# pjmikkol/bwtc

Measured on NVIDIA B200. Metric: forward BWT MB/s (SA+BWT, 32 MiB blocks), higher is better.
Workload: dtype u8 text / u32 ranks / u64 sort keys (integer)

## Files before the change

### bwtc_b200/__init__.py

```python
from __future__ import annotations

import ctypes
import os
from typing import List, Optional, Sequence

import numpy as np

_HERE = os.path.dirname(os.path.abspath(__file__))
LIB_PATH = os.path.join(_HERE, "libbwtc_cuda.so")
GEN_LIB_PATH = os.path.join(_HERE, "libbwtc_gen.so")
INTEGRATION_LIB_PATH = os.path.join(_HERE, "libbwtc_integration.so")

MAX_ROUNDS = 40
MAX_BLOCK = 0x7FFFFFFD
SCRATCH_BYTES_PER_SUFFIX = 40
SCRATCH_FIXED_BYTES = 8 << 20
ECORRUPT = -6
EVERIFY = -7
FLAG_VERIFIED = 1 << 6
FLAG_CORRUPT = 1 << 7
FLAG_SA = 1 << 8


class BwtcCudaUnavailable(RuntimeError):
    """The CUDA engine library is not built / not loadable.  There is no fallback path."""


class BwtcCudaError(RuntimeError):
    def __init__(self, code: int, msg: str, blocks: Optional[List[int]] = None):
        super().__init__(f"bwtc_cuda error {code}: {msg}")
        self.code = code
        self.blocks = blocks


class Stats(ctypes.Structure):

    _fields_ = [
        ("n_suffixes", ctypes.c_uint32),
        ("sigma", ctypes.c_uint32),
        ("bits_per_char", ctypes.c_uint32),
        ("chars_round0", ctypes.c_uint32),
        ("key_bytes_round0", ctypes.c_uint32),
        ("rounds", ctypes.c_uint32),
        ("live", ctypes.c_uint32 * MAX_ROUNDS),
        ("passes", ctypes.c_uint32 * MAX_ROUNDS),
        ("prefix_len", ctypes.c_uint32 * MAX_ROUNDS),
        ("kernel_launches", ctypes.c_uint64),
        ("algorithmic_bytes", ctypes.c_uint64),
        ("gpu_ms", ctypes.c_float),
        ("sort_ms", ctypes.c_float),
        ("sort_bytes", ctypes.c_uint64),
        ("sort_launches", ctypes.c_uint32),
        ("sort0_launches", ctypes.c_uint32),
        ("sort0_bytes", ctypes.c_uint64),
        ("sort0_ms", ctypes.c_float),
        ("flags", ctypes.c_uint32),
        ("batch_blocks", ctypes.c_uint32),
    ]

    def as_dict(self) -> dict:
        r = int(self.rounds)
        return {
            "n_suffixes": int(self.n_suffixes), "sigma": int(self.sigma), "bits_per_char": int(self.bits_per_char),
            "chars_round0": int(self.chars_round0), "key_bytes_round0": int(self.key_bytes_round0), "rounds": r,
            "live": [int(self.live[i]) for i in range(r)], "passes": [int(self.passes[i]) for i in range(r)],
            "prefix_len": [int(self.prefix_len[i]) for i in range(r)],
            "kernel_launches": int(self.kernel_launches), "algorithmic_bytes": int(self.algorithmic_bytes),
            "gpu_ms": float(self.gpu_ms), "sort_ms": float(self.sort_ms), "sort_bytes": int(self.sort_bytes),
            "sort_launches": int(self.sort_launches), "sort0_launches": int(self.sort0_launches),
            "sort0_bytes": int(self.sort0_bytes), "sort0_ms": float(self.sort0_ms), "flags": int(self.flags),
            "batch_blocks": int(self.batch_blocks),
        }


# ... 517 lines not shown
```

### bwtc_b200/csrc/bwt_engine.cu

```cuda
#include "../../include/bwtc_cuda.h"
#include "bwt_kernels.cuh"
#include "ibwt_kernels.cuh"

#include <algorithm>
#include <atomic>
#include <chrono>
#include <cmath>
#include <condition_variable>
#include <cstdarg>
#include <cstdio>
#include <cstdlib>
#include <cstring>
#include <deque>
#include <memory>
#include <mutex>
#include <thread>
#include <unordered_map>
#include <vector>

using namespace bwtc_b200;

namespace {

constexpr int RS_BLOCK = BWTC_RS_BLOCK;
// ... 48 lines not shown
  int wait_mode = 0;
  uint32_t cap = 0;
  size_t max_rs_tiles = 0, max_aux_tiles = 0;
  uint8_t* d_in = nullptr;
  uint8_t* d_text = nullptr;
  uint8_t* d_out = nullptr;
  uint32_t* d_rank = nullptr;
  void* d_keys[2] = {nullptr, nullptr};
  uint32_t* d_idx[2] = {nullptr, nullptr};
  uint8_t* d_aux[2] = {nullptr, nullptr};
  uint32_t* d_scat = nullptr;
  uint32_t* d_zero = nullptr;
  uint32_t* d_status = nullptr;
  uint32_t* d_tilecnt = nullptr;
  uint32_t* d_LF = nullptr;
  uint32_t* d_livebits = nullptr;
  uint32_t* d_ktab = nullptr;
  LookupParams* d_lookup = nullptr;
  LookupParams* h_lookup = nullptr;
  LadderState* d_state = nullptr;
  LadderState* h_state = nullptr;
  unsigned long long* d_wtab = nullptr;
  uint32_t* d_bhist = nullptr;
  const uint8_t** d_bptr = nullptr;
  int32_t* d_sa = nullptr;
  uint32_t* h_small = nullptr;
  uint8_t* h_batch = nullptr;
  cudaEvent_t ev_begin = nullptr, ev_end = nullptr;
  std::vector<cudaEvent_t> ev_pool;
  int timing_detail = 0;
  int static_tiles = 1;
  int lb_watchdog = 0;
  int debug_fake_watchdog = 0;
  int debug_reverse_tiles = 0;
  int verify = 0;
  int debug_corrupt_out = 0;
  uint32_t debug_corrupt_lf = 0;
  int64_t debug_corrupt_sa = -1;
  int d2h_kernel = 0;
  int d2h_ctas = 16;
  int debug_skip_copies = 0;
  int ladder_first = 2, ladder_more = 4;
  int use_radix9 = 0;
  uint32_t status_row_words = 256;
  int use_partial = 1;
  int use_gram = 1;
  int twopass = 0;
  int hybrid2 = 0;
  uint32_t rerank_pf_tiles = 0;
  int use_lazy = 1;
  uint32_t lazy_min_suffixes = 4u << 20;
  double lazy_max_live = 0.09;
  double lazy_max_repeats = 32.0;
  int use_seg = 1;
  int use_batch = 1;
  int use_pack_pred = 1;
  uint32_t aux_min_suffixes = 96u << 20;
  int bucket_min_windows = 3;
  uint64_t rerank_window_bytes = 72ull << 20;
  uint32_t force_chars = 0, force_keybytes = 0;
  uint32_t debug_max_rounds = 0;
  int last_cur = 0;
  RerankParams rr0;
  bwtc_cuda_stats stats;
  char err[512];
  uint32_t* d_ctrl() const { return d_zero; }
  uint32_t* d_hist() const { return d_zero + CTR_WORDS; }
  unsigned long long* d_tstate() const { return reinterpret_cast<unsigned long long*>(d_zero + CTR_WORDS + HIST_WORDS); }
  uint32_t* h_ctrl() const { return h_small; }
  uint32_t* h_hist() const { return h_small + CTR_WORDS; }
  uint32_t* h_LF() const { return h_small + CTR_WORDS + HIST_WORDS; }
};

#define CK(ctx, call)                                                                              \
  do {                                                                                             \
    cudaError_t e_ = (call);                                                                       \
    if (e_ != cudaSuccess) {                                                                       \
      set_err((ctx)->err, "CUDA error %s at %s:%d: %s", cudaGetErrorName(e_), __FILE__, __LINE__,  \
              cudaGetErrorString(e_));                                                             \
      return BWTC_CUDA_ECUDA;                                                                      \
    }                                                                                              \
  } while (0)

namespace {

template <typename KeyT, int IPT, bool IOTA, bool AUX, int RB = 8>
int set_pass_attr(bwtc_cuda_ctx* ctx) {
  CK(ctx, cudaFuncSetAttribute(k_radix_pass<KeyT, RS_BLOCK, IPT, IOTA, AUX, RB>, cudaFuncAttributeMaxDynamicSharedMemorySize,
                               (int)RadixPassSmem<KeyT, RS_BLOCK, IPT, AUX, RB>::bytes));
  return 0;
}

void ctx_free(bwtc_cuda_ctx* c) {
  if (!c) return;
  cudaSetDevice(c->device);
  if (c->stream) cudaStreamSynchronize(c->stream);
  cudaFree(c->d_in); cudaFree(c->d_text); cudaFree(c->d_out); cudaFree(c->d_rank);
  cudaFree(c->d_keys[0]); cudaFree(c->d_keys[1]); cudaFree(c->d_idx[0]); cudaFree(c->d_idx[1]);
  cudaFree(c->d_zero); cudaFree(c->d_status); cudaFree(c->d_LF); cudaFree(c->d_wtab); cudaFree(c->d_tilecnt); cudaFree(c->d_scat);
  cudaFree(c->d_bhist); cudaFree(c->d_bptr); cudaFree(c->d_aux[0]); cudaFree(c->d_aux[1]);
  cudaFree(c->d_state); cudaFree(c->d_livebits); cudaFree(c->d_ktab); cudaFree(c->d_lookup); cudaFree(c->d_sa);
  if (c->h_lookup) cudaFreeHost(c->h_lookup);
  if (c->h_batch) cudaFreeHost(c->h_batch);
  if (c->h_small) cudaFreeHost(c->h_small);
  if (c->h_state) cudaFreeHost(c->h_state);
  if (c->h_ring) cudaFreeHost(c->h_ring);
// ... 57 lines not shown
      chars = cmax64;
      for (uint32_t c = 1; c <= cmax64; ++c) {
        const double p0 = std::ceil(((double)c * b + blk_bits) / 8.0) * ((uint64_t)c * b + blk_bits > 32 ? 1.1 : 1.0);
        const double L = 1.0 - std::exp(-(double)N * std::exp2(-H0 * (double)c));
        const double cost = p0 + L * (npd + 2.0);
        if (cost < best - 1e-9) { best = cost; chars = c; }
      }
      const uint32_t np = div_up((uint64_t)chars * b + blk_bits, 8);
      const uint32_t cfull = (8 * np - blk_bits) / b;
      const uint32_t cap = ((uint64_t)chars * b + blk_bits <= 32) ? cmax32 : cmax64;
      chars = cfull < cap ? cfull : cap;
      keybytes = ((uint64_t)chars * b + blk_bits <= 32) ? 4 : 8;
    }
  }
  pl->has_memory = true;
  pl->live_pred = 1.0;
  pl->repeats = HUGE_VAL;
  if (!(ctx->force_chars || ctx->force_keybytes)) {
    double q2 = 0.0;
    for (int c = 0; c < 256; ++c)
      if (present[c] && count[c]) { const double q = (double)count[c] / total; q2 += q * q; }
    const double samples = pair_stats[1];
    const double all_pairs = samples * (samples - 1.0) * 0.5;
    const double expected = all_pairs * std::pow(q2, 8.0);
    pl->has_memory = (H0 < 1e-3) || samples < 64.0 || (pair_stats[0] > 8.0 * expected + 16.0);
    if (!pl->has_memory) pl->live_pred = 1.0 - std::exp(-(double)N * std::exp2(-H0 * (double)chars));
    if (samples >= 64.0) pl->repeats = pair_stats[0] / all_pairs * (double)N;
  }
  pl->sigma = sigma;
  pl->bits = b;
  pl->chars = chars;
  pl->keybytes = keybytes;
  pl->npass = div_up((uint64_t)chars * b + blk_bits, 8);
  pl->rb = 8;
  if (ctx->use_radix9 && keybytes == 8 && div_up((uint64_t)chars * b + blk_bits, 9) < pl->npass) {
    pl->rb = 9;
    pl->npass = div_up((uint64_t)chars * b + blk_bits, 9);
  }
  {
    const uint32_t covered = std::min<uint32_t>(pl->rb * pl->npass, keybytes * 8u);
    const uint32_t used = chars * b + blk_bits;
    uint32_t r = (ctx->use_partial && blk_bits == 0 && covered > used) ? covered - used : 0u;
    if (r >= b) r = b - 1u;
    if (chars >= 64u) r = 0;
    pl->rbits = r;
  }
  pl->pp.rbits = pl->rbits;
  pl->pp.bits = b;
  pl->pp.chars = chars;
  pl->pp.nblocks = 1;
  pl->pp.stride = 0;
}

uint32_t rerank_windows(const bwtc_cuda_ctx* ctx, uint32_t N, uint32_t m) {
  if ((uint64_t)m * 4 < (uint64_t)N) return 1;
  uint64_t w = ((uint64_t)N * 4 + ctx->rerank_window_bytes - 1) / ctx->rerank_window_bytes;
  if (w < 1) w = 1;
  if (!ctx->bucket_min_windows && w > 8) w = 8;
  if (w > MAX_RERANK_WINDOWS) w = MAX_RERANK_WINDOWS;
  return (uint32_t)w;
}

uint32_t rerank_launches(const bwtc_cuda_ctx* ctx, uint32_t N, uint32_t m) {
  const uint32_t w = rerank_windows(ctx, N, m);
  return (ctx->bucket_min_windows && w >= (uint32_t)ctx->bucket_min_windows) ? 1u : w;
}

inline bool dbg_any(const bwtc_cuda_ctx* ctx) { return ctx->debug_max_rounds != 0; }

inline uint32_t tile_slot(const bwtc_cuda_ctx* ctx, uint32_t ticket_word) {
  if (!ctx->static_tiles) return ticket_word;
  return ctx->debug_reverse_tiles ? CTR_STATIC_REV : CTR_STATIC;
}

inline uint32_t* status_rows(const bwtc_cuda_ctx* ctx, int p) {
  return ctx->d_status + ((size_t)p * (ctx->max_rs_tiles + LB_PAD_ROWS) + LB_PAD_ROWS) * ctx->status_row_words;
}

struct PassTimer {
  bwtc_cuda_ctx* ctx;
  size_t used = 0;
  int begin() {
    if (!ctx->timing_detail) return 0;
    if (used + 2 > ctx->ev_pool.size()) return 0;
    CK(ctx, cudaEventRecord(ctx->ev_pool[used], ctx->stream));
    return 0;
  }
  int end() {
    if (!ctx->timing_detail) return 0;
    if (used + 2 > ctx->ev_pool.size()) return 0;
    CK(ctx, cudaEventRecord(ctx->ev_pool[used + 1], ctx->stream));
    used += 2;
    return 0;
  }
};

template <typename KeyT, int IPT, bool AUX, int RB = 8>
int run_sort_impl(bwtc_cuda_ctx* ctx, uint32_t m, uint32_t pass_mask, bool first_iota, uint32_t iota_top, int* cur_io,
                  PassTimer* pt, uint32_t* passes_done, uint32_t pack_bits, uint32_t topshift, uint32_t pred_mask) {
  constexpr uint32_t TILE = RS_BLOCK * IPT;
  const uint32_t tiles = div_up(m, TILE);
  const size_t smem = RadixPassSmem<KeyT, RS_BLOCK, IPT, AUX, RB>::bytes;
  int cur = *cur_io;
  bool iota = first_iota;
  uint32_t done = 0;
  for (int p = 0; p < MAX_PASSES; ++p) {
// ... 391 lines not shown
  } else {
    const uint8_t last = J.h_in ? J.h_in[N - 1] : *h_last;
    J.last = last;
    J.present[last] = true;
    count[last] += 1;
  }
  double pair_stats[2];
  memcpy(pair_stats, ctx->h_LF() + 256, 16);
  plan_round0(ctx, count, J.present, N, pair_stats, &J.pl, J.blk_bits);
  if (bs) { J.pl.pp.nblocks = bs->nblocks; J.pl.pp.stride = J.bstride; }
  J.ep.nblocks = bs ? bs->nblocks : 1u;
  J.ep.stride = J.bstride;
  J.ep.text = J.d_text;
  J.ep.out = J.d_dst;
  J.ep.lastch = ctx->d_LF + LF_PARK;
  J.ep.N = N;
  J.ep.block_mode = J.block_mode ? 1 : 0;
  J.ep.sa = J.sa;
  S.sigma = J.pl.sigma;
  S.bits_per_char = J.pl.bits;
  S.chars_round0 = J.pl.chars;
  S.key_bytes_round0 = J.pl.keybytes;
  J.a_launches = S.kernel_launches;
  J.a_bytes = S.algorithmic_bytes;
  return 0;
}

int verify_forward(bwtc_cuda_ctx* ctx, const Job& J);
int verify_sa(bwtc_cuda_ctx* ctx, const Job& J);

int64_t phase_sort(bwtc_cuda_ctx* ctx, Job& J) {
  ctx->lb_watchdog = 0;
  if (cudaSetDevice(ctx->device) != cudaSuccess) {
    set_err(ctx->err, "cudaSetDevice(%d) failed", ctx->device);
    return BWTC_CUDA_ECUDA;
  }
  cudaStream_t st = ctx->stream;
  bwtc_cuda_stats& S = ctx->stats;
  const BatchSpec* bs = J.bs;
  const uint32_t N = J.N, n = J.n;
  const Round0Plan& pl = J.pl;
  const EmitParams& ep = J.ep;
  const uint8_t* d_text = J.d_text;
  PassTimer pt{ctx};
  S.kernel_launches = J.a_launches;
  S.algorithmic_bytes = J.a_bytes;
  S.sort_bytes = S.sort0_bytes = 0;
  S.sort_launches = S.sort0_launches = 0;
  CK(ctx, cudaMemsetAsync(ctx->d_zero, 0, (size_t)CTR_STICKY * 4, st));
  CK(ctx, cudaMemsetAsync(ctx->d_state, 0, sizeof(LadderState), st));
  CK(ctx, cudaMemsetAsync(ctx->d_LF + LF_PARK, 0, (size_t)(LF_WORDS - LF_PARK) * 4, st));

  const uint32_t rs_tile0 = pl.keybytes == 4 ? RS_TILE32 : RS_TILE64;
  const uint32_t all0 = (1u << pl.npass) - 1u;
  if (zero_round_state(ctx, N, N, rs_tile0, all0, pl.rb)) return BWTC_CUDA_ECUDA;
  {
    const uint32_t ptiles = div_up(N, AUX_TILE);
    const int grid = (int)(ptiles < (uint32_t)(ctx->sm_count * 4) ? ptiles : (uint32_t)(ctx->sm_count * 4));
    uint32_t hist_mask = 0;
    DeriveParams dp;
    dp.count = 0;
    const uint32_t keybits = pl.chars * pl.bits;
    const uint32_t rbits = pl.rbits;
    uint32_t regular_mask = 0;
    for (uint32_t p = 0; p < pl.npass; ++p) {
      int rep = -1;
      const uint32_t rb = pl.rb;
      const bool full_p = (rb * p >= rbits) && (rb * p - rbits + rb <= keybits);
      if (full_p) regular_mask |= 1u << p;
      if (full_p && N > 64 && !bs)
        for (uint32_t r = 0; r < p; ++r)
          if (((hist_mask >> r) & (regular_mask >> r) & 1u) && (rb * (p - r)) % pl.bits == 0) { rep = (int)r; break; }
      if (rep < 0) {
        hist_mask |= 1u << p;
      } else {
        dp.p[dp.count] = (uint8_t)p;
        dp.r[dp.count] = (uint8_t)rep;
        dp.t[dp.count] = (uint8_t)(pl.rb * (p - (uint32_t)rep) / pl.bits);
        dp.count++;
      }
    }
    GramParams gp;
    gp.npass = 0;
    bool use_gram = ctx->use_gram && !bs && N > 64 && (pl.bits == 6 || pl.bits == 3) && keybits >= (uint32_t)GRAM_BITS;
    if (use_gram) {
      const uint32_t W = (uint32_t)GRAM_BITS / pl.bits;
      for (uint32_t p = 0; p < pl.npass && use_gram; ++p) {
        uint32_t u, sft;
        gp.next[p] = 0;
        if (pl.rb * p < rbits) {
          if (p != 0) use_gram = false;
          u = 0;
          sft = pl.bits - rbits;
          gp.next[p] = 1;
          if (sft + pl.rb > (uint32_t)GRAM_BITS) use_gram = false;
        } else {
          const uint32_t lo = pl.rb * p - rbits;
          u = std::min<uint32_t>(lo / pl.bits, pl.chars - W);
          sft = lo - pl.bits * u;
          if (sft + pl.rb > (uint32_t)GRAM_BITS && lo + pl.rb <= keybits) use_gram = false;
        }
        if (sft >= 32u) use_gram = false;
        gp.u[p] = (uint8_t)u;
        gp.s[p] = (uint8_t)sft;
      }
      gp.npass = pl.npass;
    }
    uint32_t* gram = use_gram ? ctx->d_hist() + GRAM_OFF : nullptr;
    if (use_gram) { hist_mask = 0; dp.count = 0; }
    if (pl.keybytes == 4) {
      k_pack_round0<uint32_t><<<grid, 256, 0, st>>>(d_text, N, static_cast<uint32_t*>(ctx->d_keys[0]), pl.pp,
                                                     ctx->d_hist(), hist_mask, ptiles, pl.rb, gram);
      if (dp.count) k_hist_derive<uint32_t><<<dp.count, 256, 0, st>>>(d_text, N, pl.pp, dp, ctx->d_hist(), pl.rb);
      if (use_gram) k_hist_from_gram<uint32_t><<<gp.npass, 256, 0, st>>>(d_text, N, pl.pp, gp, gram, ctx->d_hist(), pl.rb);
    } else {
      k_pack_round0<unsigned long long><<<grid, 256, 0, st>>>(d_text, N, static_cast<unsigned long long*>(ctx->d_keys[0]),
                                                               pl.pp, ctx->d_hist(), hist_mask, ptiles, pl.rb, gram);
      if (dp.count) k_hist_derive<unsigned long long><<<dp.count, 256, 0, st>>>(d_text, N, pl.pp, dp, ctx->d_hist(), pl.rb);
      if (use_gram)
        k_hist_from_gram<unsigned long long><<<gp.npass, 256, 0, st>>>(d_text, N, pl.pp, gp, gram, ctx->d_hist(), pl.rb);
    }
    if (dp.count || use_gram) S.kernel_launches++;
    CK(ctx, cudaGetLastError());
    S.kernel_launches++;
    S.algorithmic_bytes += (uint64_t)N + (uint64_t)N * pl.keybytes;
  }
  const uint32_t mask0 = all0;
  int cur = 0;
  uint32_t pdone = 0;
  int rc;
  uint32_t id_bits = (uint32_t)ceil_log2_u64((uint64_t)N);
  if (id_bits < 1) id_bits = 1;
  const bool pack_pred = ctx->use_pack_pred && (id_bits + pl.bits <= 32) && (mask0 & 1u);
  const uint32_t topshift = (pl.chars - 1) * pl.bits + pl.rbits;
  const uint32_t pred_mask = (1u << pl.bits) - 1u;
  const bool aux_pred = !pack_pred && ctx->aux_min_suffixes && N >= ctx->aux_min_suffixes && (mask0 & 1u) && !bs;
  if (pl.keybytes == 4)
    rc = run_sort<uint32_t, RS_IPT32>(ctx, N, mask0, true, N - 1, &cur, &pt, &pdone, pack_pred ? id_bits : 0u, topshift,
                                      pred_mask, aux_pred);
  else
    rc = run_sort<unsigned long long, RS_IPT64>(ctx, N, mask0, true, N - 1, &cur, &pt, &pdone, pack_pred ? id_bits : 0u,
                                                topshift, pred_mask, aux_pred, pl.rb);
  if (rc) return rc;
  const size_t round0_events = pt.used;
  S.sort0_launches = S.sort_launches;
  S.sort0_bytes = S.sort_bytes;
  S.live[0] = N;
  S.passes[0] = pdone;
  S.prefix_len[0] = 0;
  S.rounds = 1;
  bool lazy = false;
  const uint32_t keybits0 = pl.chars * pl.bits + pl.rbits;
  if (ctx->use_lazy && !bs && !dbg_any(ctx) && N >= 64 && keybits0 >= 1) {
    constexpr uint32_t LAZY_MIN_CHARS = 10;
    const bool memory_ok = ctx->use_seg && pl.chars >= LAZY_MIN_CHARS && pl.repeats <= ctx->lazy_max_repeats;
    lazy = ctx->use_lazy >= 2 ||
           (N >= ctx->lazy_min_suffixes && (pl.has_memory ? memory_ok : pl.live_pred <= ctx->lazy_max_live));
  }
  const uint32_t tbits = std::min<uint32_t>(KTAB_BITS, keybits0);
  const uint32_t lazy_cap = N / 6;
  {
    RerankParams rp;
    rp.m = N;
    {
      const uint32_t text_end = J.sentinel_outside_alphabet ? N - 1 : N;
      const uint32_t wchars = pl.chars + (pl.rbits ? 1u : 0u);
      rp.short_thresh = wchars > text_end ? 0u : text_end - wchars + 1u;
    }
    rp.lo_bits = 0;
    rp.lazy = lazy ? 1u : 0u;
    rp.livebits = ctx->d_livebits;
    rp.ktab = ctx->d_ktab;
    rp.tshift = keybits0 - tbits;
    if (lazy) {
      CK(ctx, cudaMemsetAsync(ctx->d_livebits, 0, ((size_t)N / 32 + 4) * 4, st));
      CK(ctx, cudaMemsetAsync(ctx->d_ktab, 0xFF, ((size_t)(1u << tbits) + 2) * 4, st));
      LookupParams& L = *ctx->h_lookup;
      L.enabled = 1;
      L.keybytes = pl.keybytes;
      L.sorted_keys = ctx->d_keys[cur];
      L.ktab = ctx->d_ktab;
      L.livebits = ctx->d_livebits;
      L.text = d_text;
      L.N = N;
      L.bits = pl.bits;
      L.chars = pl.chars;
      L.rbits = pl.rbits;
      L.tshift = keybits0 - tbits;
      memcpy(L.lut, pl.pp.lut, 256);
      CK(ctx, cudaMemcpyAsync(ctx->d_lookup, ctx->h_lookup, sizeof(LookupParams), cudaMemcpyHostToDevice, st));
    }
    S.flags = (ctx->static_tiles ? 0u : 1u) | (bs ? 2u : 0u) | (pack_pred ? 4u : 0u) | (aux_pred ? 8u : 0u) | (lazy ? 16u : 0u) |
              (J.sa ? 256u : 0u);
    rp.packed = pack_pred ? 1u : (aux_pred ? 2u : 0u);
    rp.pred_aux = ctx->d_aux[cur];
    rp.id_bits = pack_pred ? id_bits : 31u;
    rp.id_mask = pack_pred ? (uint32_t)((1ull << id_bits) - 1ull) : 0xFFFFFFFFu;
    memset(rp.decode, 0, sizeof(rp.decode));
    for (int c = 0; c < 256; ++c)
      if (J.present[c]) rp.decode[pl.pp.lut[c]] = (uint8_t)c;
    uint32_t* snr = reinterpret_cast<uint32_t*>(ctx->d_keys[cur ^ 1]);
    if (pl.keybytes == 4) rc = launch_rerank<uint32_t, true>(ctx, cur, N, N, rp, ep, snr, snr + N, lazy);
    else rc = launch_rerank<unsigned long long, true>(ctx, cur, N, N, rp, ep, snr, snr + N, lazy);
    if (rc) return rc;
    S.algorithmic_bytes += (uint64_t)N * (pl.keybytes + 4) + (lazy ? 0ull : (uint64_t)N * 4);
    if (lazy) {
      const uint32_t entries = 1u << tbits, nchunks = div_up(entries, KTAB_CHUNK);
      uint32_t* cmin = ctx->d_bhist;
      k_ktab_chunkmin<<<nchunks, 256, 0, st>>>(ctx->d_ktab, entries, cmin);
      k_ktab_fill<<<nchunks, 256, 0, st>>>(ctx->d_ktab, entries, N, cmin, nchunks);
      CK(ctx, cudaGetLastError());
      S.kernel_launches += 2;
    }
    ctx->rr0 = rp;
  }
  PoolPtrs pool;
  pool.p[0] = reinterpret_cast<uint32_t*>(ctx->d_keys[0]);
  pool.p[1] = reinterpret_cast<uint32_t*>(ctx->d_keys[0]) + N;
  pool.p[2] = reinterpret_cast<uint32_t*>(ctx->d_keys[1]);
  pool.p[3] = reinterpret_cast<uint32_t*>(ctx->d_keys[1]) + N;
  pool.p[4] = ctx->d_idx[0];
  pool.p[5] = ctx->d_idx[1];
  const PoolPtrs norm = pool;
  if (lazy) {
    for (int q = 0; q < 6; ++q) pool.p[q] = ctx->d_scat + (size_t)q * lazy_cap;
  }
  const LookupParams* lkp = lazy ? ctx->d_lookup : nullptr;
  ctx->last_cur = cur;
  uint32_t m_prev = N;
  uint32_t m_bound = N;
  uint64_t h_next = pl.chars;
  auto sel_of = [&lazy](int c) { return lazy ? 0x10u : ((uint32_t)(2 * c) | ((uint32_t)(2 * c + 1) << 4)); };
  k_commit_sort<<<1, 1, 0, st>>>(ctx->d_state, ctx->d_ctrl(), (uint32_t)std::min<uint64_t>(h_next, 0x7FFFFFFFull), sel_of(cur),
                                 0xFFFFFFFFu, 1u, lazy ? lazy_cap : 0xFFFFFFFFu);
  S.kernel_launches++;

  auto make_lists = [&](bool speculative) -> int {
    const uint32_t tiles = div_up(m_prev, AUX_TILE);
    k_scan_tile_counts<<<1, 1024, 0, st>>>(ctx->d_tilecnt, ctx->d_tilecnt + ctx->max_aux_tiles, tiles);
    k_gather_chunks<<<tiles, 256, 0, st>>>(norm.p[2 * (cur ^ 1)], norm.p[2 * (cur ^ 1) + 1], ctx->d_tilecnt,
                                           ctx->d_tilecnt + ctx->max_aux_tiles, AUX_TILE, lazy ? pool.p[0] : norm.p[2 * cur],
                                           lazy ? pool.p[1] : norm.p[2 * cur + 1], speculative ? ctx->d_state : nullptr,
                                           ctx->d_ctrl());
    CK(ctx, cudaGetLastError());
    S.kernel_launches += 2;
    return 0;
// ... 784 lines not shown
  }
  return n;
}

#define BWTC_STR2(x) #x
#define BWTC_STR(x) BWTC_STR2(x)
const char* bwtc_cuda_version(void) {
  return "bwtc_b200 0.1 sm_100a radix-pass BLOCK=" BWTC_STR(BWTC_RS_BLOCK) " IPT64=" BWTC_STR(BWTC_RS_IPT64)
         " IPT32=" BWTC_STR(BWTC_RS_IPT32);
}

const char* bwtc_cuda_global_error(void) { return g_err; }

uint32_t bwtc_cuda_stats_sizeof(void) { return (uint32_t)sizeof(bwtc_cuda_stats); }

int bwtc_cuda_ctx_create(bwtc_cuda_ctx** out, int device, uint32_t max_block_bytes) {
  if (!out || max_block_bytes == 0) { set_err(g_err, "bad arguments"); return BWTC_CUDA_EARG; }
  if (max_block_bytes > BWTC_CUDA_MAX_BLOCK) { set_err(g_err, "max_block_bytes above engine limit"); return BWTC_CUDA_ETOOBIG; }
  *out = nullptr;
  cudaError_t e = cudaSetDevice(device);
  if (e != cudaSuccess) { set_err(g_err, "cudaSetDevice(%d): %s", device, cudaGetErrorString(e)); return BWTC_CUDA_ECUDA; }
  bwtc_cuda_ctx* c = new (std::nothrow) bwtc_cuda_ctx();
  if (!c) { set_err(g_err, "out of host memory"); return BWTC_CUDA_EALLOC; }
  c->device = device;
  c->cap = max_block_bytes;
  if (const char* e = getenv("BWTC_STATIC_TILES")) c->static_tiles = atoi(e);
  if (const char* e = getenv("BWTC_DEBUG_FAKE_WATCHDOG")) c->debug_fake_watchdog = atoi(e);
  if (const char* e = getenv("BWTC_DEBUG_REVERSE_TILES")) c->debug_reverse_tiles = atoi(e);
  if (const char* e = getenv("BWTC_VERIFY")) c->verify = atoi(e) ? 1 : 0;
  if (const char* e = getenv("BWTC_DEBUG_CORRUPT_OUT")) c->debug_corrupt_out = atoi(e);
  if (const char* e = getenv("BWTC_DEBUG_CORRUPT_LF")) c->debug_corrupt_lf = (uint32_t)std::max(0, atoi(e));
  if (const char* e = getenv("BWTC_DEBUG_CORRUPT_SA")) c->debug_corrupt_sa = std::max(-1L, atol(e));
  if (const char* e = getenv("BWTC_DEBUG_SKIP_COPIES")) c->debug_skip_copies = atoi(e);
  if (const char* e = getenv("BWTC_D2H_KERNEL")) c->d2h_kernel = atoi(e);
  if (const char* e = getenv("BWTC_D2H_CTAS")) c->d2h_ctas = std::max(1, atoi(e));
  if (const char* e = getenv("BWTC_SPIN_WAIT")) c->wait_mode = atoi(e) ? 1 : 0;
  if (const char* e = getenv("BWTC_WAIT_MODE")) c->wait_mode = atoi(e);
  if (const char* e = getenv("BWTC_POLL_SPIN_US")) c->poll_spin_us = std::max(0, atoi(e));
  if (const char* e = getenv("BWTC_POLL_SLEEP_US")) c->poll_sleep_us = std::max(1, atoi(e));
  if (const char* e = getenv("BWTC_LADDER_FIRST")) c->ladder_first = std::max(0, atoi(e));
  if (const char* e = getenv("BWTC_LADDER_MORE")) c->ladder_more = std::max(1, atoi(e));
  if (const char* e = getenv("BWTC_LAZY")) c->use_lazy = atoi(e);
  if (const char* e = getenv("BWTC_HYBRID2")) c->hybrid2 = atoi(e);
  if (const char* e = getenv("BWTC_TWOPASS")) c->twopass = atoi(e);
  if (const char* e = getenv("BWTC_GRAM")) c->use_gram = atoi(e);
  if (const char* e = getenv("BWTC_PARTIAL")) c->use_partial = atoi(e);
  if (const char* e = getenv("BWTC_RERANK_PF")) c->rerank_pf_tiles = (uint32_t)std::max(0, atoi(e));
  c->use_radix9 = env_radix9();
  c->status_row_words = status_row_words_for(c->use_radix9);
  if (const char* e = getenv("BWTC_LAZY_MIN_MIB")) c->lazy_min_suffixes = (uint32_t)std::max(0L, atol(e)) << 20;
  if (const char* e = getenv("BWTC_LAZY_MAX_LIVE")) c->lazy_max_live = atof(e);
  if (const char* e = getenv("BWTC_LAZY_MAX_REPEATS")) c->lazy_max_repeats = atof(e);
  if (const char* e = getenv("BWTC_SEG")) c->use_seg = atoi(e);
  if (const char* e = getenv("BWTC_BATCH")) c->use_batch = atoi(e);
  if (const char* e = getenv("BWTC_PACK_PRED")) c->use_pack_pred = atoi(e);
  if (const char* e = getenv("BWTC_AUX_MIN_MIB")) { const long v = atol(e); c->aux_min_suffixes = v > 0 ? (uint32_t)v << 20 : (v == 0 ? 1u : 0u); }
  if (const char* e = getenv("BWTC_BUCKET_MIN_WINDOWS")) c->bucket_min_windows = atoi(e);
  if (const char* e = getenv("BWTC_RERANK_WINDOW_MB")) { long v = atol(e); if (v > 0) c->rerank_window_bytes = (uint64_t)v << 20; }
  c->err[0] = 0;
  memset(&c->stats, 0, sizeof(c->stats));
  const size_t N = (size_t)max_block_bytes + 1;
  const uint32_t min_tile = RS_TILE64 < RS_TILE32 ? RS_TILE64 : RS_TILE32;
  c->max_rs_tiles = div_up(N, min_tile);
  c->max_aux_tiles = div_up(N, AUX_TILE);
  int rc = 0;
#define ALLOC(ptr, bytes)                                                                       \
  do {                                                                                          \
    if (!rc) {                                                                                  \
      e = cudaMalloc((void**)&(ptr), (bytes));                                                  \
      if (e != cudaSuccess) {                                                                   \
        set_err(g_err, "cudaMalloc(%zu bytes) for " #ptr ": %s", (size_t)(bytes), cudaGetErrorString(e)); \
        rc = BWTC_CUDA_EALLOC;                                                                  \
      }                                                                                         \
    }                                                                                           \
  } while (0)
  int sm = 0;
  if (cudaDeviceGetAttribute(&sm, cudaDevAttrMultiProcessorCount, device) == cudaSuccess && sm > 0) c->sm_count = sm;
  {
    size_t free_b = 0, total_b = 0;
    const uint64_t need = bwtc_cuda_scratch_bytes(max_block_bytes);
    if (cudaMemGetInfo(&free_b, &total_b) == cudaSuccess && need > (uint64_t)free_b) {
      set_err(g_err, "a context for %u-byte blocks needs %llu bytes of device memory, %llu are free", max_block_bytes,
              (unsigned long long)need, (unsigned long long)free_b);
      delete c;
      return BWTC_CUDA_EALLOC;
    }
  }
  e = cudaStreamCreateWithFlags(&c->stream, cudaStreamNonBlocking);
  if (e != cudaSuccess) { set_err(g_err, "cudaStreamCreate: %s", cudaGetErrorString(e)); rc = BWTC_CUDA_ECUDA; }
  const size_t padded = ((N + TEXT_PAD + 15) / 16) * 16 + 16;
  ALLOC(c->d_in, padded);
  ALLOC(c->d_text, padded);
  ALLOC(c->d_out, padded);
  ALLOC(c->d_rank, (N + 64) * 4);
  ALLOC(c->d_keys[0], N * 8 + 64);
  ALLOC(c->d_keys[1], N * 8 + 64);
  ALLOC(c->d_idx[0], N * 4);
  ALLOC(c->d_idx[1], N * 4);
  ALLOC(c->d_zero, (size_t)(CTR_WORDS + HIST_WORDS) * 4 + (size_t)MAX_RERANK_WINDOWS * c->max_aux_tiles * 8 + 64);
  ALLOC(c->d_status, (size_t)MAX_PASSES * (c->max_rs_tiles + LB_PAD_ROWS) * c->status_row_words * 4u);
  ALLOC(c->d_LF, (size_t)LF_WORDS * 4);
  ALLOC(c->d_state, sizeof(LadderState));
  ALLOC(c->d_livebits, (N / 32 + 4) * 4);
  ALLOC(c->d_ktab, ((size_t)(1u << KTAB_BITS) + 2) * 4);
  ALLOC(c->d_lookup, sizeof(LookupParams));
  ALLOC(c->d_bhist, (size_t)MAX_BATCH * 256 * 4);
// ... 628 lines not shown
```

### bwtc_b200/csrc/bwt_kernels.cuh

```cuda
#pragma once
#include <cuda_runtime.h>
#include <stdint.h>

namespace bwtc_b200 {

constexpr uint32_t RANK_DONE = 0x80000000u;
constexpr uint32_t RANK_MASK = 0x7FFFFFFFu;

constexpr int CTR_ERR = 0;
constexpr int CTR_STICKY = 8;
constexpr int CTR_PASS0 = 8;
constexpr uint32_t CTR_STATIC = 0xFFFFFFFFu;
constexpr uint32_t CTR_STATIC_REV = 0xFFFFFFFEu;
constexpr int CTR_CURSOR = 24;
constexpr int CTR_LIVE = 25;
constexpr int CTR_MAXGROUP = 26;
constexpr int CTR_UPD = 27;
constexpr int CTR_RERANK = 32;
constexpr int MAX_RERANK_WINDOWS = 16;
constexpr int CTR_WORDS = 64;

constexpr uint32_t LB_PREFIX = 0x80000000u, LB_VALUE = 0x7FFFFFFFu;
constexpr uint32_t LB_PAD_WORD = LB_PREFIX | 1u;
__constant__ uint32_t g_lb_spin_limit = 1u << 24;
// ... 344 lines not shown
#pragma unroll
          for (int k = 0; k < IPT; k += 2) dst[k / 2] = make_ulonglong2((unsigned long long)out[k], (unsigned long long)out[k + 1]);
        } else {
          uint4* dst = reinterpret_cast<uint4*>(keys + t);
#pragma unroll
          for (int k = 0; k < IPT; k += 4)
            dst[k / 4] = make_uint4((uint32_t)out[k], (uint32_t)out[k + 1], (uint32_t)out[k + 2], (uint32_t)out[k + 3]);
        }
      } else {
#pragma unroll
        for (int k = 0; k < IPT; ++k)
          if (t + k < N) keys[t + k] = out[k];
      }
      if (gram) {
#pragma unroll
        for (int k = 0; k < IPT; ++k)
          if (t + k < N) atomicAdd(&s_hist[(uint32_t)(out[k] >> pp.rbits) & ((1u << GRAM_BITS) - 1u)], 1u);
      } else {
#pragma unroll
        for (int k = 0; k < IPT; ++k) {
          if (t + k < N) {
#pragma unroll
            for (int p = 0; p < (int)(sizeof(KeyT)); ++p)
              if ((hist_mask >> p) & 1u) atomicAdd(&s_hist[(p << rb) + ((uint32_t)(out[k] >> (rb * p)) & dmask)], 1u);
          }
        }
      }
    }
    __syncthreads();
  }
  if (gram) {
    for (uint32_t e = tid; e < (1u << GRAM_BITS); e += BLOCK) {
      const uint32_t v = s_hist[e];
      if (v) atomicAdd(&gram[e], v);
    }
    return;
  }
#pragma unroll
  for (int p = 0; p < (int)(sizeof(KeyT)); ++p) {
    if (!((hist_mask >> p) & 1u)) continue;
    for (uint32_t e = tid; e <= dmask; e += BLOCK) {
      const uint32_t v = s_hist[(p << rb) + e];
      if (v) atomicAdd(&hist[(p << rb) + e], v);
    }
  }
}

struct DeriveParams {
  uint32_t count;
  uint8_t p[8], r[8], t[8];
};

struct GramParams {
  uint32_t npass;
  uint8_t u[8], s[8];
  uint8_t next[8];
};

template <typename KeyT>
__device__ __forceinline__ KeyT pack_key_at(const uint8_t* __restrict__ text, uint32_t N, uint32_t i, const uint8_t* lut,
                                            uint32_t b, uint32_t c, uint32_t rbits) {
  KeyT key = 0;
  for (uint32_t j = 0; j < c; ++j) {
    const uint32_t g = i + j;
    key = (KeyT)(key << b) | (KeyT)((g < N) ? lut[text[g]] : 0u);
  }
  if (rbits) {
    const uint32_t g = i + c;
    key = (KeyT)(key << rbits) | (KeyT)(((g < N) ? (uint32_t)lut[text[g]] : 0u) >> (b - rbits));
  }
  return key;
}

template <typename KeyT>
__global__ void __launch_bounds__(256) k_hist_derive(const uint8_t* __restrict__ text, uint32_t N, PackParams pp,
                                                     DeriveParams dp, uint32_t* __restrict__ hist, uint32_t rb) {
  __shared__ uint8_t s_lut[256];
  __shared__ uint32_t s_h[512];
  const int tid = threadIdx.x;
  const uint32_t p = dp.p[blockIdx.x], r = dp.r[blockIdx.x], t = dp.t[blockIdx.x];
  const uint32_t dmask = (1u << rb) - 1u;
  s_lut[tid] = pp.lut[tid];
  for (uint32_t e = tid; e <= dmask; e += 256) s_h[e] = hist[(r << rb) + e];
  __syncthreads();
  if ((uint32_t)tid < t) {
    if ((uint32_t)tid < N) {
      const KeyT kh = pack_key_at<KeyT>(text, N, (uint32_t)tid, s_lut, pp.bits, pp.chars, pp.rbits);
      atomicAdd(&s_h[(uint32_t)(kh >> (rb * p)) & dmask], 1u);
    }
    if ((uint32_t)tid < N) {
      const KeyT kt = pack_key_at<KeyT>(text, N, N - 1u - (uint32_t)tid, s_lut, pp.bits, pp.chars, pp.rbits);
      atomicSub(&s_h[(uint32_t)(kt >> (rb * r)) & dmask], 1u);
    }
  }
  __syncthreads();
  for (uint32_t e = tid; e <= dmask; e += 256) hist[(p << rb) + e] = s_h[e];
}

template <typename KeyT>
__global__ void __launch_bounds__(256) k_hist_from_gram(const uint8_t* __restrict__ text, uint32_t N, PackParams pp,
                                                        GramParams gp, const uint32_t* __restrict__ gram,
                                                        uint32_t* __restrict__ hist, uint32_t rb) {
  __shared__ uint8_t s_lut[256];
  __shared__ uint32_t s_h[512];
  const int tid = threadIdx.x;
  const uint32_t p = blockIdx.x, u = gp.u[p], sh = gp.s[p];
  const uint32_t dmask = (1u << rb) - 1u;
  s_lut[tid] = pp.lut[tid];
  s_h[tid] = 0;
  s_h[tid + 256] = 0;
  __syncthreads();
  for (uint32_t g = tid; g < (1u << GRAM_BITS); g += 256) {
    const uint32_t v = gram[g];
    if (v) atomicAdd(&s_h[(g >> sh) & dmask], v);
  }
  if (gp.next[p]) {
    if (tid == 0) {
      const KeyT k0 = pack_key_at<KeyT>(text, N, 0u, s_lut, pp.bits, pp.chars, pp.rbits);
      atomicSub(&s_h[(((uint32_t)(k0 >> pp.rbits) & ((1u << GRAM_BITS) - 1u)) >> sh) & dmask], 1u);
      atomicAdd(&s_h[0], 1u);
    }
  } else if ((uint32_t)tid < u && (uint32_t)tid < N) {
    const KeyT kh = pack_key_at<KeyT>(text, N, (uint32_t)tid, s_lut, pp.bits, pp.chars, pp.rbits);
    atomicAdd(&s_h[(uint32_t)(kh >> (rb * p)) & dmask], 1u);
    const KeyT kt = pack_key_at<KeyT>(text, N, N - 1u - (uint32_t)tid, s_lut, pp.bits, pp.chars, pp.rbits);
    atomicSub(&s_h[(((uint32_t)(kt >> pp.rbits) & ((1u << GRAM_BITS) - 1u)) >> sh) & dmask], 1u);
  }
  __syncthreads();
  for (uint32_t e = tid; e <= dmask; e += 256) hist[(p << rb) + e] = s_h[e];
}

__global__ void __launch_bounds__(256) k_build_keys(const uint32_t* __restrict__ rank, uint32_t N, uint32_t h,
                                                    int lo_bits, unsigned long long* __restrict__ keys,
                                                    uint32_t* __restrict__ idx, uint32_t* __restrict__ ctrl,
                                                    uint32_t* __restrict__ hist, int npass, uint32_t ntiles,
                                                    uint32_t rb) {
  constexpr int BLOCK = 256, IPT = 8, TILE = BLOCK * IPT, WARPS = BLOCK / 32;
  __shared__ uint32_t s_hist[8 * 512];
  __shared__ uint32_t s_wtot[WARPS];
  __shared__ uint32_t s_base;
  const int tid = threadIdx.x, lane = tid & 31, warp = tid >> 5;
  const uint32_t dmask = (1u << rb) - 1u;
  if (ctrl[CTR_ERR]) return;
#pragma unroll
  for (int p = 0; p < 16; ++p) s_hist[p * 256 + tid] = 0;
  __syncthreads();
  for (uint32_t tile = blockIdx.x; tile < ntiles; tile += gridDim.x) {
    const uint32_t i0 = tile * (uint32_t)TILE + tid * IPT;
    uint32_t r[IPT];
    {
      const uint4* pr = reinterpret_cast<const uint4*>(rank + i0);
      uint4 a = make_uint4(RANK_DONE, RANK_DONE, RANK_DONE, RANK_DONE), b4 = a;
      if (i0 < N) a = pr[0];
      if (i0 + 4 < N) b4 = pr[1];
      r[0] = a.x; r[1] = a.y; r[2] = a.z; r[3] = a.w;
      r[4] = b4.x; r[5] = b4.y; r[6] = b4.z; r[7] = b4.w;
    }
    uint32_t livemask = 0;
#pragma unroll
// ... 351 lines not shown
#pragma unroll
        for (int i = 0; i < LB_BATCH; ++i) v[i] = ld_relaxed_u32(row - i * 256);
        uint32_t alive = 0xFFFFFFFFu, fin = 0;
        int consumed = 0;
#pragma unroll
        for (int i = 0; i < LB_BATCH; ++i) {
          const uint32_t pubd = (uint32_t)((int32_t)(v[i] | (0u - v[i])) >> 31);
          const uint32_t ispre = (uint32_t)((int32_t)v[i] >> 31);
          const uint32_t isagg = pubd & ~ispre;
          excl += ((v[i] & LB_VALUE) - 1u) & alive & pubd;
          fin |= alive & ispre;
          consumed += (int)(alive & isagg & 1u);
          alive &= isagg;
        }
        done = fin != 0;
        t -= consumed;
        if (!done && consumed == 0) {
          ++spins;
          if (spins > g_lb_spin_limit || ((spins & 255u) == 0u && ld_relaxed_u32(ctrl + CTR_ERR))) {
            atomicExch(&ctrl[CTR_ERR], 1u);
            break;
          }
          __nanosleep(20);
        }
      }
      st_relaxed_u32(my_status, LB_PREFIX | ((excl + pub + 1u) & LB_VALUE));
#ifdef BWTC_PROFILE_STAGES
      if (tid == 0 && g_prof_buf) {
        g_prof_buf[(size_t)tile * 16 + 9] = prof_iters;
        g_prof_buf[(size_t)tile * 16 + 10] = spins;
        g_prof_buf[(size_t)tile * 16 + 11] = clock64();
        g_prof_buf[(size_t)tile * 16 + 12] = (unsigned long long)((long long)tile - 1 - t);
      }
#endif
    }
    s_binbase[tid] = gexcl + excl - texcl;
  }
  __syncthreads();
  BWTC_PROF(6);
#pragma unroll
  for (int k = 0; k < IPT; ++k) {
    const uint32_t p = tid + k * BLOCK;
    const KeyT kk = s_keys[p];
    const uint32_t vv = s_vals[p];
    const uint32_t d = (uint32_t)(kk >> shift) & 0xFFu;
    const uint32_t g = s_binbase[d] + p;
    if (p < valid) {
      BWTC_ST(keys_out + g, kk);
      BWTC_ST(vals_out + g, vv);
      if (AUX) aux_out[g] = s_aux[p];
    }
  }
  BWTC_PROF(8);
}

struct RerankParams {
  uint32_t m;
  uint32_t short_thresh;
  int lo_bits;
  uint32_t win_lo, win_hi;
  uint32_t ctr_slot;
  uint32_t id_mask;
  uint32_t id_bits;
  uint32_t packed;
  const uint8_t* pred_aux;
  uint8_t decode[256];
  uint32_t nbuckets;
  uint32_t bucket_magic;
  uint32_t* nr_out;
  uint32_t direct0;
  uint32_t lazy;
  uint32_t emit;
  uint32_t pf_tiles;
  uint32_t* livebits;
  uint32_t* ktab;
  uint32_t tshift;
};

struct LookupParams {
  uint32_t enabled;
  uint32_t keybytes;
  const void* sorted_keys;
  const uint32_t* ktab;
  const uint32_t* livebits;
  const uint8_t* text;
  uint32_t N, bits, chars, tshift;
  uint32_t rbits;
  uint8_t lut[256];
};

template <typename KeyT>
__device__ __forceinline__ uint32_t sector_lower_bound(const KeyT* __restrict__ sk, KeyT key, uint32_t lo, uint32_t hi,
                                                       uint32_t frac16) {
  constexpr uint32_t KPS = 32 / sizeof(KeyT);
  uint32_t g = lo + (uint32_t)(((unsigned long long)(hi - lo) * frac16) >> 16);
  for (int it = 0; lo < hi; ++it) {
    if (g >= hi) g = hi - 1u;
    if (g < lo) g = lo;
    const uint32_t s = g & ~(KPS - 1u);
    KeyT v[KPS];
    if constexpr (sizeof(KeyT) == 8) {
      const ulonglong2 x = *reinterpret_cast<const ulonglong2*>(sk + s);
      const ulonglong2 y = *reinterpret_cast<const ulonglong2*>(sk + s + 2);
      v[0] = (KeyT)x.x; v[1] = (KeyT)x.y; v[2] = (KeyT)y.x; v[3] = (KeyT)y.y;
    } else {
      const uint4 x = *reinterpret_cast<const uint4*>(sk + s);
// ... 1340 lines not shown
```

Baseline: 14850.

## Split round-0 radix sort: skip low 16-bit passes and finish ties per group

Measured after the change: 9908 (median of 6 runs). 0.667x the previous value.

```diff
diff --git a/bwtc_b200/__init__.py b/bwtc_b200/__init__.py
--- a/bwtc_b200/__init__.py
+++ b/bwtc_b200/__init__.py
@@ -20,6 +20,7 @@
 FLAG_VERIFIED = 1 << 6
 FLAG_CORRUPT = 1 << 7
 FLAG_SA = 1 << 8
+FLAG_SPLIT0 = 1 << 9
 
 
 class BwtcCudaUnavailable(RuntimeError):
diff --git a/bwtc_b200/csrc/bwt_engine.cu b/bwtc_b200/csrc/bwt_engine.cu
--- a/bwtc_b200/csrc/bwt_engine.cu
+++ b/bwtc_b200/csrc/bwt_engine.cu
@@ -124,6 +124,7 @@
   uint32_t lazy_min_suffixes = 4u << 20;
   double lazy_max_live = 0.09;
   double lazy_max_repeats = 32.0;
+  int use_split0 = 1;
   int use_seg = 1;
   int use_batch = 1;
   int use_pack_pred = 1;
@@ -287,6 +288,14 @@
   pl->pp.stride = 0;
 }
 
+bool split_round0(const bwtc_cuda_ctx* ctx, const Round0Plan& pl, bool batch) {
+  constexpr double SPLIT0_MAX_REPEATS = 32.0;
+  if (!ctx->use_split0 || batch || pl.keybytes != 8 || pl.rb != 8 || pl.npass * 8u <= (uint32_t)SPLIT_LO_BITS) return false;
+  if (ctx->use_split0 >= 2) return true;
+  return pl.has_memory && pl.bits * 8u <= 64u - (uint32_t)SPLIT_LO_BITS && pl.npass == 8 &&
+         pl.repeats <= SPLIT0_MAX_REPEATS;
+}
+
 uint32_t rerank_windows(const bwtc_cuda_ctx* ctx, uint32_t N, uint32_t m) {
   if ((uint64_t)m * 4 < (uint64_t)N) return 1;
   uint64_t w = ((uint64_t)N * 4 + ctx->rerank_window_bytes - 1) / ctx->rerank_window_bytes;
@@ -784,8 +793,10 @@
   CK(ctx, cudaMemsetAsync(ctx->d_LF + LF_PARK, 0, (size_t)(LF_WORDS - LF_PARK) * 4, st));
 
   const uint32_t rs_tile0 = pl.keybytes == 4 ? RS_TILE32 : RS_TILE64;
-  const uint32_t all0 = (1u << pl.npass) - 1u;
-  if (zero_round_state(ctx, N, N, rs_tile0, all0, pl.rb)) return BWTC_CUDA_ECUDA;
+  const bool split0 = split_round0(ctx, pl, bs != nullptr);
+  const uint32_t first0 = split0 ? (uint32_t)SPLIT_LO_BITS / pl.rb : 0u;
+  const uint32_t mask0 = ((1u << pl.npass) - 1u) & ~((1u << first0) - 1u);
+  if (zero_round_state(ctx, N, N, rs_tile0, mask0, pl.rb)) return BWTC_CUDA_ECUDA;
   {
     const uint32_t ptiles = div_up(N, AUX_TILE);
     const int grid = (int)(ptiles < (uint32_t)(ctx->sm_count * 4) ? ptiles : (uint32_t)(ctx->sm_count * 4));
@@ -795,7 +806,7 @@
     const uint32_t keybits = pl.chars * pl.bits;
     const uint32_t rbits = pl.rbits;
     uint32_t regular_mask = 0;
-    for (uint32_t p = 0; p < pl.npass; ++p) {
+    for (uint32_t p = first0; p < pl.npass; ++p) {
       int rep = -1;
       const uint32_t rb = pl.rb;
       const bool full_p = (rb * p >= rbits) && (rb * p - rbits + rb <= keybits);
@@ -814,10 +825,11 @@
     }
     GramParams gp;
     gp.npass = 0;
+    gp.first = 0;
     bool use_gram = ctx->use_gram && !bs && N > 64 && (pl.bits == 6 || pl.bits == 3) && keybits >= (uint32_t)GRAM_BITS;
     if (use_gram) {
       const uint32_t W = (uint32_t)GRAM_BITS / pl.bits;
-      for (uint32_t p = 0; p < pl.npass && use_gram; ++p) {
+      for (uint32_t p = first0; p < pl.npass && use_gram; ++p) {
         uint32_t u, sft;
         gp.next[p] = 0;
         if (pl.rb * p < rbits) {
@@ -836,6 +848,7 @@
         gp.u[p] = (uint8_t)u;
         gp.s[p] = (uint8_t)sft;
       }
+      gp.first = first0;
       gp.npass = pl.npass;
     }
     uint32_t* gram = use_gram ? ctx->d_hist() + GRAM_OFF : nullptr;
@@ -844,29 +857,28 @@
       k_pack_round0<uint32_t><<<grid, 256, 0, st>>>(d_text, N, static_cast<uint32_t*>(ctx->d_keys[0]), pl.pp,
                                                      ctx->d_hist(), hist_mask, ptiles, pl.rb, gram);
       if (dp.count) k_hist_derive<uint32_t><<<dp.count, 256, 0, st>>>(d_text, N, pl.pp, dp, ctx->d_hist(), pl.rb);
-      if (use_gram) k_hist_from_gram<uint32_t><<<gp.npass, 256, 0, st>>>(d_text, N, pl.pp, gp, gram, ctx->d_hist(), pl.rb);
+      if (use_gram) k_hist_from_gram<uint32_t><<<gp.npass - gp.first, 256, 0, st>>>(d_text, N, pl.pp, gp, gram, ctx->d_hist(), pl.rb);
     } else {
       k_pack_round0<unsigned long long><<<grid, 256, 0, st>>>(d_text, N, static_cast<unsigned long long*>(ctx->d_keys[0]),
                                                                pl.pp, ctx->d_hist(), hist_mask, ptiles, pl.rb, gram);
       if (dp.count) k_hist_derive<unsigned long long><<<dp.count, 256, 0, st>>>(d_text, N, pl.pp, dp, ctx->d_hist(), pl.rb);
       if (use_gram)
-        k_hist_from_gram<unsigned long long><<<gp.npass, 256, 0, st>>>(d_text, N, pl.pp, gp, gram, ctx->d_hist(), pl.rb);
+        k_hist_from_gram<unsigned long long><<<gp.npass - gp.first, 256, 0, st>>>(d_text, N, pl.pp, gp, gram, ctx->d_hist(), pl.rb);
     }
     if (dp.count || use_gram) S.kernel_launches++;
     CK(ctx, cudaGetLastError());
     S.kernel_launches++;
     S.algorithmic_bytes += (uint64_t)N + (uint64_t)N * pl.keybytes;
   }
-  const uint32_t mask0 = all0;
   int cur = 0;
   uint32_t pdone = 0;
   int rc;
   uint32_t id_bits = (uint32_t)ceil_log2_u64((uint64_t)N);
   if (id_bits < 1) id_bits = 1;
-  const bool pack_pred = ctx->use_pack_pred && (id_bits + pl.bits <= 32) && (mask0 & 1u);
+  const bool pack_pred = ctx->use_pack_pred && (id_bits + pl.bits <= 32);
   const uint32_t topshift = (pl.chars - 1) * pl.bits + pl.rbits;
   const uint32_t pred_mask = (1u << pl.bits) - 1u;
-  const bool aux_pred = !pack_pred && ctx->aux_min_suffixes && N >= ctx->aux_min_suffixes && (mask0 & 1u) && !bs;
+  const bool aux_pred = !pack_pred && ctx->aux_min_suffixes && N >= ctx->aux_min_suffixes && !bs;
   if (pl.keybytes == 4)
     rc = run_sort<uint32_t, RS_IPT32>(ctx, N, mask0, true, N - 1, &cur, &pt, &pdone, pack_pred ? id_bits : 0u, topshift,
                                       pred_mask, aux_pred);
@@ -874,6 +886,18 @@
     rc = run_sort<unsigned long long, RS_IPT64>(ctx, N, mask0, true, N - 1, &cur, &pt, &pdone, pack_pred ? id_bits : 0u,
                                                 topshift, pred_mask, aux_pred, pl.rb);
   if (rc) return rc;
+  if (split0) {
+    unsigned long long* keys = static_cast<unsigned long long*>(ctx->d_keys[cur]);
+    uint8_t* aux = aux_pred ? ctx->d_aux[cur] : nullptr;
+    k_group_finish<unsigned long long><<<div_up(N, GF_TILE), GF_BLOCK, 0, st>>>(keys, ctx->d_idx[cur], aux, N, ctx->d_ctrl(),
+                                                                              ctx->d_idx[cur ^ 1]);
+    k_group_finish_big<unsigned long long><<<ctx->sm_count, 256, 0, st>>>(
+        keys, ctx->d_idx[cur], aux, N, ctx->d_ctrl(), ctx->d_idx[cur ^ 1],
+        static_cast<unsigned long long*>(ctx->d_keys[cur ^ 1]), aux_pred ? ctx->d_aux[cur ^ 1] : nullptr);
+    CK(ctx, cudaGetLastError());
+    S.kernel_launches += 2;
+    S.algorithmic_bytes += (uint64_t)N * pl.keybytes;
+  }
   const size_t round0_events = pt.used;
   S.sort0_launches = S.sort_launches;
   S.sort0_bytes = S.sort_bytes;
@@ -923,7 +947,7 @@
       CK(ctx, cudaMemcpyAsync(ctx->d_lookup, ctx->h_lookup, sizeof(LookupParams), cudaMemcpyHostToDevice, st));
     }
     S.flags = (ctx->static_tiles ? 0u : 1u) | (bs ? 2u : 0u) | (pack_pred ? 4u : 0u) | (aux_pred ? 8u : 0u) | (lazy ? 16u : 0u) |
-              (J.sa ? 256u : 0u);
+              (J.sa ? 256u : 0u) | (split0 ? 512u : 0u);
     rp.packed = pack_pred ? 1u : (aux_pred ? 2u : 0u);
     rp.pred_aux = ctx->d_aux[cur];
     rp.id_bits = pack_pred ? id_bits : 31u;
@@ -1814,6 +1838,7 @@
   if (const char* e = getenv("BWTC_LAZY_MAX_LIVE")) c->lazy_max_live = atof(e);
   if (const char* e = getenv("BWTC_LAZY_MAX_REPEATS")) c->lazy_max_repeats = atof(e);
   if (const char* e = getenv("BWTC_SEG")) c->use_seg = atoi(e);
+  if (const char* e = getenv("BWTC_SPLIT0")) c->use_split0 = atoi(e);
   if (const char* e = getenv("BWTC_BATCH")) c->use_batch = atoi(e);
   if (const char* e = getenv("BWTC_PACK_PRED")) c->use_pack_pred = atoi(e);
   if (const char* e = getenv("BWTC_AUX_MIN_MIB")) { const long v = atol(e); c->aux_min_suffixes = v > 0 ? (uint32_t)v << 20 : (v == 0 ? 1u : 0u); }
diff --git a/bwtc_b200/csrc/bwt_kernels.cuh b/bwtc_b200/csrc/bwt_kernels.cuh
--- a/bwtc_b200/csrc/bwt_kernels.cuh
+++ b/bwtc_b200/csrc/bwt_kernels.cuh
@@ -420,7 +420,7 @@
 };
 
 struct GramParams {
-  uint32_t npass;
+  uint32_t first, npass;
   uint8_t u[8], s[8];
   uint8_t next[8];
 };
@@ -472,7 +472,7 @@
   __shared__ uint8_t s_lut[256];
   __shared__ uint32_t s_h[512];
   const int tid = threadIdx.x;
-  const uint32_t p = blockIdx.x, u = gp.u[p], sh = gp.s[p];
+  const uint32_t p = gp.first + blockIdx.x, u = gp.u[p], sh = gp.s[p];
   const uint32_t dmask = (1u << rb) - 1u;
   s_lut[tid] = pp.lut[tid];
   s_h[tid] = 0;
@@ -930,6 +930,154 @@
     }
   }
   BWTC_PROF(8);
+}
+
+constexpr int SPLIT_LO_BITS = 16;
+constexpr int GF_BLOCK = 256, GF_TILE = 2048, GF_CAP = 256;
+constexpr int GF_ITEMS = (GF_TILE + GF_CAP + GF_BLOCK - 1) / GF_BLOCK;
+constexpr int CTR_BIGRUN = 28;
+
+template <typename KeyT>
+__global__ void __launch_bounds__(GF_BLOCK) k_group_finish(KeyT* __restrict__ keys, uint32_t* __restrict__ ids,
+                                                          uint8_t* __restrict__ aux, uint32_t n,
+                                                          uint32_t* __restrict__ ctrl, uint32_t* __restrict__ big) {
+  constexpr KeyT LOMASK = ((KeyT)1 << SPLIT_LO_BITS) - 1;
+  constexpr uint16_t NONE = 0xFFFFu;
+  __shared__ KeyT s_key[GF_TILE + GF_CAP + 2];
+  __shared__ uint32_t s_id[GF_TILE + GF_CAP];
+  __shared__ uint16_t s_src[GF_TILE + GF_CAP];
+  __shared__ uint8_t s_aux[GF_TILE + GF_CAP];
+  if (ctrl[CTR_ERR]) return;
+  const int tid = threadIdx.x;
+  const uint32_t t0 = blockIdx.x * (uint32_t)GF_TILE;
+  const uint32_t base = t0 ? t0 - 1u : 0u;
+  const uint32_t end = min(n, t0 + (uint32_t)(GF_TILE + GF_CAP + 1));
+  const uint32_t lim = min(n, t0 + (uint32_t)(GF_TILE + GF_CAP));
+  for (uint32_t g = base + tid; g < end; g += GF_BLOCK) s_key[g - base] = keys[g];
+  for (uint32_t g = t0 + tid; g < lim; g += GF_BLOCK) {
+    s_id[g - t0] = ids[g];
+    s_src[g - t0] = NONE;
+    if (aux) s_aux[g - t0] = aux[g];
+  }
+  __syncthreads();
+#pragma unroll
+  for (int k = 0; k < GF_ITEMS; ++k) {
+    const uint32_t p = t0 + (uint32_t)(k * GF_BLOCK + tid);
+    if (p >= lim) continue;
+    const KeyT kp = s_key[p - base], hp = kp >> SPLIT_LO_BITS;
+    const bool prev_eq = p > 0 && (s_key[p - 1 - base] >> SPLIT_LO_BITS) == hp;
+    const bool next_eq = p + 1 < end && (s_key[p + 1 - base] >> SPLIT_LO_BITS) == hp;
+    if (!prev_eq && !next_eq) continue;
+    uint32_t s = p;
+    bool owned = true;
+    while (s > 0 && (s_key[s - 1 - base] >> SPLIT_LO_BITS) == hp) {
+      if (s == t0 || p - s >= (uint32_t)GF_CAP) { owned = false; break; }
+      --s;
+    }
+    if (!owned || s >= t0 + (uint32_t)GF_TILE) continue;
+    uint32_t e = p + 1;
+    while (e < end && e - s <= (uint32_t)GF_CAP && (s_key[e - base] >> SPLIT_LO_BITS) == hp) ++e;
+    if (e - s > (uint32_t)GF_CAP) {
+      if (p == s) big[atomicAdd(&ctrl[CTR_BIGRUN], 1u)] = s;
+      continue;
+    }
+    const uint32_t lo = (uint32_t)(kp & LOMASK);
+    uint32_t r = 0;
+    for (uint32_t q = s; q < e; ++q) {
+      const uint32_t lq = (uint32_t)(s_key[q - base] & LOMASK);
+      r += (lq < lo || (lq == lo && q < p)) ? 1u : 0u;
+    }
+    if (s + r != p) s_src[s + r - t0] = (uint16_t)(p - t0);
+  }
+  __syncthreads();
+  for (uint32_t g = t0 + tid; g < lim; g += GF_BLOCK) {
+    const uint32_t q = s_src[g - t0];
+    if (q == NONE) continue;
+    keys[g] = s_key[t0 + q - base];
+    ids[g] = s_id[q];
+    if (aux) aux[g] = s_aux[q];
+  }
+}
+
+template <typename KeyT>
+__global__ void __launch_bounds__(256) k_group_finish_big(KeyT* __restrict__ keys, uint32_t* __restrict__ ids,
+                                                         uint8_t* __restrict__ aux, uint32_t n,
+                                                         const uint32_t* __restrict__ ctrl, const uint32_t* __restrict__ big,
+                                                         unsigned long long* __restrict__ tmp, uint8_t* __restrict__ tmp_aux) {
+  static_assert(SPLIT_LO_BITS == 16, "two 8-bit counting passes");
+  constexpr KeyT LOMASK = ((KeyT)1 << SPLIT_LO_BITS) - 1;
+  constexpr uint32_t FULL = 0xFFFFFFFFu;
+  __shared__ uint32_t s_h[8][2][256];
+  if (ctrl[CTR_ERR]) return;
+  const int lane = threadIdx.x & 31, warp = threadIdx.x >> 5;
+  const uint32_t lt = lanemask_lt();
+  uint32_t* h0 = s_h[warp][0];
+  uint32_t* h1 = s_h[warp][1];
+  const uint32_t nbig = ctrl[CTR_BIGRUN];
+  for (uint32_t w = blockIdx.x * 8u + (uint32_t)warp; w < nbig; w += gridDim.x * 8u) {
+    const uint32_t s = big[w];
+    const KeyT hk = keys[s] >> SPLIT_LO_BITS;
+    uint32_t e = s + (uint32_t)GF_CAP + 1u;
+    for (;; e += 32) {
+      const uint32_t g = e + (uint32_t)lane;
+      const uint32_t b = __ballot_sync(FULL, g < n && (keys[g] >> SPLIT_LO_BITS) == hk);
+      if (b != FULL) { e += (uint32_t)(__ffs(~b) - 1); break; }
+    }
+    for (int i = lane; i < 512; i += 32) s_h[warp][0][i] = 0;
+    __syncwarp();
+    for (uint32_t g = s + lane; g < e; g += 32) {
+      const uint32_t lo = (uint32_t)(keys[g] & LOMASK);
+      atomicAdd(&h0[lo & 255u], 1u);
+      atomicAdd(&h1[lo >> 8], 1u);
+    }
+    __syncwarp();
+    for (int d = 0; d < 2; ++d) {
+      uint32_t* h = s_h[warp][d];
+      uint32_t v[8], sum = 0;
+#pragma unroll
+      for (int i = 0; i < 8; ++i) { v[i] = h[lane * 8 + i]; sum += v[i]; }
+      uint32_t incl = sum;
+#pragma unroll
+      for (int o = 1; o < 32; o <<= 1) {
+        const uint32_t t = __shfl_up_sync(FULL, incl, o);
+        if (lane >= o) incl += t;
+      }
+      uint32_t run = incl - sum;
+#pragma unroll
+      for (int i = 0; i < 8; ++i) { h[lane * 8 + i] = run; run += v[i]; }
+    }
+    __syncwarp();
+    for (uint32_t b0 = s; b0 < e; b0 += 32) {
+      const uint32_t g = b0 + (uint32_t)lane;
+      const uint32_t act = __ballot_sync(FULL, g < e);
+      if (g < e) {
+        const uint32_t lo = (uint32_t)(keys[g] & LOMASK), d = lo & 255u;
+        const uint32_t peers = __match_any_sync(act, d);
+        const uint32_t pos = s + h0[d] + __popc(peers & lt);
+        tmp[pos] = ((unsigned long long)lo << 32) | ids[g];
+        if (aux) tmp_aux[pos] = aux[g];
+        __syncwarp(act);
+        if (lane == __ffs(peers) - 1) h0[d] += __popc(peers);
+      }
+      __syncwarp();
+    }
+    for (uint32_t b0 = s; b0 < e; b0 += 32) {
+      const uint32_t g = b0 + (uint32_t)lane;
+      const uint32_t act = __ballot_sync(FULL, g < e);
+      if (g < e) {
+        const unsigned long long r = tmp[g];
+        const uint32_t lo = (uint32_t)(r >> 32), d = lo >> 8;
+        const uint32_t peers = __match_any_sync(act, d);
+        const uint32_t pos = s + h1[d] + __popc(peers & lt);
+        keys[pos] = (KeyT)(hk << SPLIT_LO_BITS) | (KeyT)lo;
+        ids[pos] = (uint32_t)r;
+        if (aux) aux[pos] = tmp_aux[g];
+        __syncwarp(act);
+        if (lane == __ffs(peers) - 1) h1[d] += __popc(peers);
+      }
+      __syncwarp();
+    }
+  }
 }
 
 struct RerankParams {
```
